# pmgbergen/porepy

Hardware: NVIDIA H100
Metric: 3D cells/sec MPFA+MPSA assembly (higher is better)
Workload: dtype f64

## Files before the change

### porepy_b200/csrc/api.cu

```cuda
#include <cuda_runtime.h>

#include <omp.h>

#include <atomic>
#include <chrono>
#include <thread>
#include <climits>
#include <cstdio>
#include <cstdlib>
#include <cstring>
#include <string>
#include <vector>

#include "csr_build.cuh"
#include <nvtx3/nvToolsExt.h>

struct NvtxRange {
    explicit NvtxRange(const char *name) { nvtxRangePushA(name); }
    ~NvtxRange() { nvtxRangePop(); }
};

static thread_local std::string g_err;
static thread_local int64_t g_err_node = -1;
static std::atomic<int64_t> g_launches{0};

static int fail(int code, const std::string &msg) {
    g_err = msg;
    return code;
}
int pb_fail_(int code, const std::string &msg) { return fail(code, msg); }
void pb_count_launch_() { g_launches++; }

DevPool &pb_dev_pool_() {
    static DevPool *pool = new DevPool;
    return *pool;
}
extern "C" void pb_device_pool_trim(void) { pb_dev_pool_().trim(); }

extern "C" const char *pb_last_error(void) { return g_err.c_str(); }
static std::atomic<int64_t> g_alloc_calls[2];
static std::atomic<int64_t> g_alloc_ns[2];
void pb_alloc_stat_(int kind, double seconds) {
    g_alloc_calls[kind & 1]++;
    g_alloc_ns[kind & 1] += (int64_t)(seconds * 1e9);
}
extern "C" void pb_alloc_stats(double *out) {
    if (!out) return;
    out[0] = (double)g_alloc_calls[0].load(); out[1] = 1e-9 * (double)g_alloc_ns[0].load();
    out[2] = (double)g_alloc_calls[1].load(); out[3] = 1e-9 * (double)g_alloc_ns[1].load();
}
extern "C" int64_t pb_last_error_node(void) { return g_err_node; }
void pb_set_error_node_(int64_t node) { g_err_node = node; }
extern "C" int64_t pb_launch_count(void) { return g_launches.load(); }
extern "C" int pb_device_count(void) {
    int n = 0;
    if (cudaGetDeviceCount(&n) != cudaSuccess) return -1;
    return n;
}
extern "C" int pb_set_device(int device) {
    CUDA_TRY(cudaSetDevice(device));
    return PB_OK;
}

extern "C" int pb_host_alloc(uint64_t bytes, void **out) {
    if (!out) return fail(PB_EINVAL, "null pointer");
    CUDA_TRY(cudaHostAlloc(out, bytes ? bytes : 8, cudaHostAllocDefault));
    return PB_OK;
}
extern "C" void pb_host_free(void *p) {
    if (p) cudaFreeHost(p);
}

static int64_t cfg_scratch(int cfg, int n) {
    switch (cfg) {
        case 0: return Cfg0::scratch_doubles_c();
        case 1: return Cfg1::scratch_doubles_c();
        case 2: return Cfg2::scratch_doubles_c();
        case 3: return Cfg3::scratch_doubles_c();
        case 4: return Cfg4::scratch_doubles_c();
        case 5: return Cfg5::scratch_doubles_c();
        default: return n;
    }
}

static int64_t cfg_pool(int cfg, int n, int w) {
    switch (cfg) {
        case 0: return Cfg0::pool_doubles(n, w);
        case 1: return Cfg1::pool_doubles(n, w);
        case 2: return Cfg2::pool_doubles(n, w);
        case 3: return Cfg3::pool_doubles(n, w);
        case 4: return Cfg4::pool_doubles(n, w);
        case 5: return Cfg5::pool_doubles(n, w);
        default: return Cfg6::pool_doubles(n, w);
    }
}

template <class F>
static int build_classes(pb_plan *p, std::vector<NodeClass> &out, bool rows_to_solver, F size_of) {
    const HostPlan &H = p->H;
    std::vector<int32_t> lists[2 * kNumCfg];
    int64_t amax[2 * kNumCfg] = {0}, rmax[2 * kNumCfg] = {0}, smax[2 * kNumCfg] = {0};
    for (int64_t s = 0; s < H.nn; ++s) {
        int nsc = H.node_sc_ptr[s + 1] - H.node_sc_ptr[s];
        int nsf = H.node_sf_ptr[s + 1] - H.node_sf_ptr[s];
        if (nsf == 0) continue;
        if (!p->active.empty() && !p->active[s]) continue;
        int n = 0, w = 0;
        int64_t a = 0, r = 0;
        size_of(nsf, nsc, H.node_nb[s], &n, &w, &a, &r);
        int cfg = 0;
        while (cfg < kCatchAll && (n > kCfg[cfg].max_n || w > kCfg[cfg].max_w)) ++cfg;
        const int64_t scr = cfg_scratch(cfg, n);
        const int tpb = kCfg[cfg].team == 32 ? 4 : 1;
        bool glob = (size_t)(a + r + scr) * 8 * tpb > kMaxSmem;
        if (glob && (size_t)(r + scr) * 8 * tpb > kMaxSmem)
            return fail(PB_ENOTIMPL, "interaction region at node " + std::to_string(s) +
                                         " is too large for this build (" + std::to_string(nsf) +
                                         " sub-faces)");
        int key = cfg * 2 + (glob ? 1 : 0);
        lists[key].push_back((int32_t)s);
        amax[key] = std::max(amax[key], rows_to_solver ? cfg_pool(cfg, n, w) : a);
        rmax[key] = std::max(rmax[key], r);
        smax[key] = std::max(smax[key], scr);
    }
    out.clear();
    for (int key = 0; key < 2 * kNumCfg; ++key) {
        if (lists[key].empty()) continue;
        out.emplace_back();
        NodeClass &c = out.back();
        c.cfg = key / 2;
        c.a_global = key & 1;
        c.team = kCfg[c.cfg].team;
        c.n = (int)lists[key].size();
        c.a_doubles = amax[key];
        c.rest_doubles = rmax[key];
        c.scr_doubles = smax[key];
        if (!c.a_global) {
            const int tpb = c.team == 32 ? 4 : 1;
            if ((size_t)(c.a_doubles + c.rest_doubles + c.scr_doubles) * 8 * tpb > kMaxSmem) c.a_global = true;
        }
        if (!p->node_key.empty()) {
            const std::vector<uint32_t> &nk = p->node_key;
            std::stable_sort(lists[key].begin(), lists[key].end(), [&](int32_t x, int32_t y) { return nk[x] < nk[y]; });
        }
        if (c.nodes.upload(lists[key], p->stream) != cudaSuccess) return fail(PB_ECUDA, "upload of node list failed");
    }
    return PB_OK;
}

static int build_mpfa_classes(pb_plan *p) {
    const int nd = p->H.nd;
    return build_classes(p, p->mpfa_cls, false, [&](int nsf, int nsc, int nb, int *n, int *w, int64_t *a, int64_t *r) {
        *n = nsf;
        *w = mpfa_width(nd, nsf, nsc, nb);
        *a = mpfa_A_doubles(nd, nsf, nsc, nb);
        *r = mpfa_rest_doubles(nd, nsf, nsc, nb);
    });
}

__global__ void posmap_kernel(int64_t nn, const int32_t *__restrict__ row_ptr, const int32_t *__restrict__ row_ent,
                              const int32_t *__restrict__ col_ptr, const int32_t *__restrict__ col_ent,
                              const int32_t *__restrict__ ip, const int32_t *__restrict__ ix,
                              const int64_t *__restrict__ pos_ptr, int32_t *__restrict__ pos) {
    const int lane = threadIdx.x & 31;
    const int64_t warp = ((int64_t)blockIdx.x * blockDim.x + threadIdx.x) >> 5;
    const int64_t nwarps = ((int64_t)gridDim.x * blockDim.x) >> 5;
    for (int64_t s = warp; s < nn; s += nwarps) {
        const int r0 = row_ptr[s], nr = row_ptr[s + 1] - r0;
        const int c0 = col_ptr[s], ncl = col_ptr[s + 1] - c0;
        const int64_t base = pos_ptr[s];
        for (int e = lane; e < nr * ncl; e += 32) {
            const int i = e / ncl, j = e - i * ncl;
            const int r = row_ent[r0 + i], c = col_ent[c0 + j];
            int lo = ip[r], hi = ip[r + 1];
            while (lo < hi) {
                const int mid = (lo + hi) >> 1;
                if (ix[mid] < c) lo = mid + 1; else hi = mid;
            }
            pos[base + e] = lo;
        }
    }
}

extern "C" int pb_plan_create(int nd, int64_t nc, int64_t nf, int64_t nn, const int32_t *cf_indptr,
                              const int32_t *cf_indices, const int8_t *cf_data,
                              const int32_t *fn_indptr, const int32_t *fn_indices, pb_plan **out) {
    NvtxRange nvtx_("pb_plan_create");
    if (!out || !cf_indptr || !cf_indices || !cf_data || !fn_indptr || !fn_indices)
        return fail(PB_EINVAL, "null pointer");
    int ndev = 0;
    if (cudaGetDeviceCount(&ndev) != cudaSuccess || ndev < 1)
        return fail(PB_ECUDA, "no CUDA device: libporeb200 has no CPU path");
    pb_plan *p = new pb_plan;
    {
        int hw = (int)std::thread::hardware_concurrency();
        const char *lws = getenv("LOCAL_WORLD_SIZE");
        int share = hw / std::max(1, lws ? atoi(lws) : 1);
        const char *ov = getenv("POREB200_PLAN_THREADS");
        int nt = ov ? atoi(ov) : std::min(64, std::max(1, share));
        pb::g_plan_threads = std::max(1, nt);
    }
    auto tp0 = std::chrono::steady_clock::now();
    auto bail = [&](const char *what, cudaError_t e) {
        std::string m = std::string(what) + ": " + cudaGetErrorString(e);
        delete p;
        return fail(PB_ECUDA, m);
    };
    cudaError_t e;
    if ((e = cudaStreamCreateWithFlags(&p->stream, cudaStreamNonBlocking)) != cudaSuccess) return bail("stream", e);
    if ((e = cudaEventCreate(&p->e0)) != cudaSuccess) return bail("event", e);
    if ((e = cudaEventCreate(&p->e1)) != cudaSuccess) return bail("event", e);
    HostPlan &H = p->H;
    cudaStream_t st = p->stream;
    DevBuf fn_idx_dev;
    int rc = getenv("POREB200_HOST_PLAN") ? -1
             : pb_build_device_topology_(p, nd, nc, nf, nn, cf_indptr, cf_indices, cf_data, fn_indptr, fn_indices,
                                         fn_idx_dev);
    if (rc > 0) { delete p; return rc; }
    const bool device_topology = rc == 0;
    if (getenv("POREB200_PLAN_TIMING")) {
        cudaStreamSynchronize(st);
        fprintf(stderr, "[plan] topology on the %s        %8.1f ms (since start)\n", device_topology ? "device" : "host  ",
                std::chrono::duration<double, std::milli>(std::chrono::steady_clock::now() - tp0).count());
    }
    if (!device_topology) {
        p->H = HostPlan{};
        std::string err;
        rc = build_host_plan(nd, nc, nf, nn, cf_indptr, cf_indices, cf_data, fn_indptr, fn_indices,
                             p->H, err, false, false);
        if (rc) {
            delete p;
            return fail(rc, err);
        }
#define UP(field, vec)                                                      \
    if ((e = p->field.upload(vec, st)) != cudaSuccess) return bail(#field, e);
        UP(fn_indptr, H.fn_indptr) UP(node_sc_ptr, H.node_sc_ptr) UP(sc_cell, H.sc_cell)
        UP(node_sf_ptr, H.node_sf_ptr) UP(sf_face, H.sf_face) UP(sf_sides, H.sf_sides)
        UP(sf_bloc, H.sf_bloc) UP(slot_sf, H.slot_sf) UP(node_nb, H.node_nb) UP(sc_ncn, H.sc_ncn)
        UP(posfc_ptr, H.posfc_ptr) UP(posfb_ptr, H.posfb_ptr) UP(poscc_ptr, H.poscc_ptr)
        UP(poscb_ptr, H.poscb_ptr) UP(nbf_ptr, H.nbf_ptr) UP(nbf_idx, H.nbf_idx) UP(cn_ptr, H.cn_ptr)
        UP(cn_idx, H.cn_idx) UP(face_cells, H.face_cells)
#undef UP
        if ((e = fn_idx_dev.upload(fn_indices, (size_t)fn_indptr[nf], st)) != cudaSuccess) return bail("fn_indices", e);
        if ((e = p->cf_ip.upload(cf_indptr, (size_t)nc + 1, st)) != cudaSuccess) return bail("cf_indptr", e);
        if ((e = p->cf_ix.upload(cf_indices, (size_t)cf_indptr[nc], st)) != cudaSuccess) return bail("cf_indices", e);
        if ((e = p->cf_sg.upload(cf_data, (size_t)cf_indptr[nc], st)) != cudaSuccess) return bail("cf_data", e);
    }
    {
        struct PJob { int which; int64_t nrows, ncols; DevBuf *rnp, *rn, *cp, *ci; };
        PJob pj[4] = {{0, nf, nc, &p->fn_indptr, &fn_idx_dev, &p->node_sc_ptr, &p->sc_cell},
                      {1, nf, nf, &p->fn_indptr, &fn_idx_dev, &p->nbf_ptr, &p->nbf_idx},
                      {2, nc, nc, &p->cn_ptr, &p->cn_idx, &p->node_sc_ptr, &p->sc_cell},
                      {3, nc, nf, &p->cn_ptr, &p->cn_idx, &p->nbf_ptr, &p->nbf_idx}};
        DevBuf counts, flag;
        if ((e = flag.ensure(sizeof(int))) != cudaSuccess) return bail("flag", e);
        if ((e = cudaMemsetAsync(flag.p, 0, sizeof(int), st)) != cudaSuccess) return bail("memset", e);
        bool host_fallback = false;
        for (auto &j : pj) {
            DevBuf &ip = p->pat_ip[j.which];
            if ((e = counts.ensure((size_t)j.nrows * sizeof(int32_t))) != cudaSuccess) return bail("counts", e);
            if ((e = ip.ensure((size_t)(j.nrows + 1) * sizeof(int32_t))) != cudaSuccess) return bail("indptr", e);
            const int block = 256;
            int grid = (int)std::max<int64_t>(1, std::min<int64_t>((j.nrows + 7) / 8, (int64_t)pb_sm_count() * 8));
            pattern_kernel<256><<<grid, block, 0, st>>>(j.nrows, j.rnp->as<int32_t>(), j.rn->as<int32_t>(),
                                                        j.cp->as<int32_t>(), j.ci->as<int32_t>(),
                                                        counts.as<int32_t>(), nullptr, nullptr, 0, flag.as<int>());
            g_launches++;
            int ov = 0;
            if ((e = cudaMemcpyAsync(&ov, flag.p, sizeof(ov), cudaMemcpyDeviceToHost, st)) != cudaSuccess) return bail("copy", e);
            int64_t tot = 0;
            if ((rc = pb_scan_offsets_(counts.as<int32_t>(), ip.as<int32_t>(), j.nrows, st, &tot))) { delete p; return rc; }
            if (ov) { host_fallback = true; break; }
            if (tot > 0x7FFFFFFFll) { delete p; return fail(PB_EINVAL, "pattern exceeds 2^31 entries; split the grid"); }
            if ((e = p->pat_idx[j.which].ensure((size_t)std::max<int64_t>(1, tot) * sizeof(int32_t))) != cudaSuccess) return bail("indices", e);
            pattern_kernel<256><<<grid, block, 0, st>>>(j.nrows, j.rnp->as<int32_t>(), j.rn->as<int32_t>(),
                                                        j.cp->as<int32_t>(), j.ci->as<int32_t>(), nullptr,
                                                        ip.as<int32_t>(), p->pat_idx[j.which].as<int32_t>(), 1,
                                                        flag.as<int>());
            g_launches++;
            p->pat_rows[j.which] = j.nrows; p->pat_cols[j.which] = j.ncols; p->pat_nnz[j.which] = tot;
        }
        if (host_fallback) {
            std::string err2;
            HostPlan H2;
            int rc2 = build_host_plan(nd, nc, nf, nn, cf_indptr, cf_indices, cf_data, fn_indptr, fn_indices,
                                      H2, err2, false, true);
            if (rc2) { delete p; return fail(rc2, err2); }
            for (int w = 0; w < 4; ++w) {
                if ((e = p->pat_ip[w].upload(H2.pat[w].indptr, st)) != cudaSuccess) return bail("indptr", e);
                if ((e = p->pat_idx[w].upload(H2.pat[w].indices, st)) != cudaSuccess) return bail("indices", e);
                p->pat_rows[w] = H2.pat[w].nrows; p->pat_cols[w] = H2.pat[w].ncols; p->pat_nnz[w] = H2.pat[w].nnz();
            }
            if ((e = cudaStreamSynchronize(st)) != cudaSuccess) return bail("sync", e);
        }
        if (getenv("POREB200_PLAN_TIMING")) {
            cudaStreamSynchronize(st);
            fprintf(stderr, "[plan] patterns on device done     %8.1f ms (since start)\n",
                    std::chrono::duration<double, std::milli>(std::chrono::steady_clock::now() - tp0).count());
        }
    }
    {
        struct Job { DevBuf *pos; const std::vector<int64_t> *ptr; DevBuf *pptr; int pat;
                     DevBuf *rp, *re, *cp, *ce; };
        Job jobs[4] = {
            {&p->pos_fc, &H.posfc_ptr, &p->posfc_ptr, 0, &p->node_sf_ptr, &p->sf_face, &p->node_sc_ptr, &p->sc_cell},
            {&p->pos_fb, &H.posfb_ptr, &p->posfb_ptr, 1, &p->node_sf_ptr, &p->sf_face, &p->nbf_ptr, &p->nbf_idx},
            {&p->pos_cc, &H.poscc_ptr, &p->poscc_ptr, 2, &p->node_sc_ptr, &p->sc_cell, &p->node_sc_ptr, &p->sc_cell},
            {&p->pos_cb, &H.poscb_ptr, &p->poscb_ptr, 3, &p->node_sc_ptr, &p->sc_cell, &p->nbf_ptr, &p->nbf_idx},
        };
        for (auto &j : jobs) {
            if ((e = j.pos->ensure((size_t)std::max<int64_t>(1, j.ptr->back()) * sizeof(int32_t))) != cudaSuccess)
                return bail("pos map", e);
            const int block = 256;
            int64_t need = (nn * 32 + block - 1) / block;
            int grid = (int)std::max<int64_t>(1, std::min<int64_t>(need, (int64_t)pb_sm_count() * 16));
            posmap_kernel<<<grid, block, 0, st>>>(nn, j.rp->as<int32_t>(), j.re->as<int32_t>(),
                                                  j.cp->as<int32_t>(), j.ce->as<int32_t>(),
                                                  p->pat_ip[j.pat].as<int32_t>(), p->pat_idx[j.pat].as<int32_t>(),
                                                  j.pptr->as<int64_t>(), j.pos->as<int32_t>());
            g_launches++;
            if ((e = cudaGetLastError()) != cudaSuccess) return bail("posmap_kernel", e);
        }
    }
    if ((e = p->err.ensure(sizeof(int))) != cudaSuccess) return bail("err", e);
    PlanView &v = p->view;
    v.nd = nd; v.nc = nc; v.nf = nf; v.nn = nn;
    v.fn_indptr = p->fn_indptr.as<int32_t>();
    v.node_sc_ptr = p->node_sc_ptr.as<int32_t>(); v.sc_cell = p->sc_cell.as<int32_t>();
    v.node_sf_ptr = p->node_sf_ptr.as<int32_t>(); v.sf_face = p->sf_face.as<int32_t>();
    v.sf_sides = p->sf_sides.as<uint32_t>(); v.sf_bloc = p->sf_bloc.as<uint16_t>();
    v.slot_sf = p->slot_sf.as<uint16_t>(); v.node_nb = p->node_nb.as<int32_t>();
    v.sc_ncn = p->sc_ncn.as<int32_t>();
    v.posfc_ptr = p->posfc_ptr.as<int64_t>(); v.posfb_ptr = p->posfb_ptr.as<int64_t>();
    v.poscc_ptr = p->poscc_ptr.as<int64_t>(); v.poscb_ptr = p->poscb_ptr.as<int64_t>();
    v.pos_fc = p->pos_fc.as<int32_t>(); v.pos_fb = p->pos_fb.as<int32_t>();
    v.pos_cc = p->pos_cc.as<int32_t>(); v.pos_cb = p->pos_cb.as<int32_t>();
    v.fc_indptr = p->pat_ip[0].as<int32_t>(); v.fb_indptr = p->pat_ip[1].as<int32_t>();
    v.cc_indptr = p->pat_ip[2].as<int32_t>(); v.cb_indptr = p->pat_ip[3].as<int32_t>();
    rc = build_mpfa_classes(p);
    if (rc) { delete p; return rc; }
    if ((e = cudaStreamSynchronize(st)) != cudaSuccess) return bail("sync", e);
    {
        auto drop = [](auto &v) { v.clear(); v.shrink_to_fit(); };
        drop(H.sc_cell); drop(H.sf_face); drop(H.sf_sides); drop(H.sf_bloc); drop(H.slot_sf); drop(H.sc_ncn);
        drop(H.posfc_ptr); drop(H.posfb_ptr); drop(H.poscc_ptr); drop(H.poscb_ptr);
        drop(H.nbf_ptr); drop(H.nbf_idx); drop(H.cn_ptr); drop(H.cn_idx); drop(H.face_cells); drop(H.fn_indptr);
    }
    if (getenv("POREB200_PLAN_TIMING"))
        fprintf(stderr, "[plan] total incl. upload          %8.1f ms\n",
                std::chrono::duration<double, std::milli>(std::chrono::steady_clock::now() - tp0).count());
    *out = p;
    return PB_OK;
}

extern "C" void pb_plan_destroy(pb_plan *p) {
    if (!p) return;
    if (p->stream) cudaStreamSynchronize(p->stream);
    if (p->e0) cudaEventDestroy(p->e0);
    if (p->e1) cudaEventDestroy(p->e1);
    if (p->stream) cudaStreamDestroy(p->stream);
    delete p;
}

extern "C" int pb_plan_sizes(const pb_plan *p, int64_t *num_subcells, int64_t *num_subfaces,
                             int64_t *num_subhalffaces, int32_t *max_sf, int32_t *max_sc) {
    if (!p) return fail(PB_EINVAL, "null plan");
    if (num_subcells) *num_subcells = p->H.S;
    if (num_subfaces) *num_subfaces = p->H.U;
    if (num_subhalffaces) *num_subhalffaces = p->H.H;
    if (max_sf) *max_sf = p->H.max_nsf;
    if (max_sc) *max_sc = p->H.max_nsc;
    return PB_OK;
}

extern "C" int pb_plan_class_counts(const pb_plan *p, int kind, int64_t *counts) {
    if (!p || !counts) return fail(PB_EINVAL, "null pointer");
    if (kind != 0 && kind != 1) return fail(PB_EINVAL, "kind must be 0 (MPFA) or 1 (MPSA)");
    for (int k = 0; k < 2 * kNumCfg; ++k) counts[k] = 0;
    for (const NodeClass &c : kind == 0 ? p->mpfa_cls : p->mpsa_cls) counts[2 * c.cfg + (c.a_global ? 1 : 0)] += c.n;
    return PB_OK;
}

extern "C" int pb_plan_set_active_nodes(pb_plan *p, const uint8_t *mask) {
    if (!p) return pb_fail_(PB_EINVAL, "null plan");
    if (mask) p->active.assign(mask, mask + p->H.nn); else p->active.clear();
    p->mpsa_cls_nalpha = -1;
    int rc = build_mpfa_classes(p);
    if (rc) return rc;
    CUDA_TRY(cudaStreamSynchronize(p->stream));
    return PB_OK;
}

extern "C" int pb_plan_pattern_size(const pb_plan *p, int which, int64_t *nrows, int64_t *nnz) {
    if (!p || which < 0 || which > 3) return fail(PB_EINVAL, "bad pattern id");
    *nrows = p->pat_rows[which];
    *nnz = p->pat_nnz[which];
    return PB_OK;
}

extern "C" int pb_plan_pattern_get(const pb_plan *p, int which, int32_t *indptr, int32_t *indices) {
    if (!p || which < 0 || which > 3) return fail(PB_EINVAL, "bad pattern id");
    CUDA_TRY(cudaMemcpyAsync(indptr, p->pat_ip[which].p, (p->pat_rows[which] + 1) * sizeof(int32_t), cudaMemcpyDeviceToHost, p->stream));
    if (p->pat_nnz[which])
        CUDA_TRY(cudaMemcpyAsync(indices, p->pat_idx[which].p, p->pat_nnz[which] * sizeof(int32_t),
                                 cudaMemcpyDeviceToHost, p->stream));
    CUDA_TRY(cudaStreamSynchronize(p->stream));
    return PB_OK;
}

__global__ void expand_pattern_kernel(int64_t nrows, const int32_t *__restrict__ ip,
                                      const int32_t *__restrict__ ix, int br, int bc,
                                      int32_t *__restrict__ nip, int32_t *__restrict__ nix) {
    const int lane = threadIdx.x & 31;
    const int64_t warp = ((int64_t)blockIdx.x * blockDim.x + threadIdx.x) >> 5;
    const int64_t nwarps = ((int64_t)gridDim.x * blockDim.x) >> 5;
    for (int64_t r = warp; r < nrows; r += nwarps) {
        const int64_t b = ip[r], len = ip[r + 1] - b;
        const int64_t base = (int64_t)br * bc * b, rowlen = len * bc;
        for (int i = 0; i < br; ++i) {
            if (lane == 0) nip[r * br + i] = (int32_t)(base + i * rowlen);
            for (int64_t t = lane; t < rowlen; t += 32) {
                const int64_t q = t / bc;
                const int j = (int)(t - q * bc);
                nix[base + i * rowlen + t] = ix[b + q] * bc + j;
            }
        }
    }
    if (warp == 0 && lane == 0) nip[nrows * br] = (int32_t)((int64_t)br * bc * ip[nrows]);
}

static int expand_pattern(pb_plan *p, int which, int br, int bc, int32_t *nip, int32_t *nix) {
    const int64_t nrows = p->pat_rows[which];
    const int block = 256;
    int grid = (int)std::max<int64_t>(1, std::min<int64_t>((nrows * 32 + block - 1) / block, (int64_t)pb_sm_count() * 16));
    expand_pattern_kernel<<<grid, block, 0, p->stream>>>(nrows, p->pat_ip[which].as<int32_t>(),
                                                         p->pat_idx[which].as<int32_t>(), br, bc, nip, nix);
    g_launches++;
    CUDA_TRY(cudaGetLastError());
    return PB_OK;
}

extern "C" int pb_plan_pattern_expanded(pb_plan *p, int which, int br, int bc, int32_t *indptr,
                                        int32_t *indices) {
    if (!p || which < 0 || which > 3 || br < 1 || bc < 1 || !indptr || !indices)
        return fail(PB_EINVAL, "bad arguments");
    struct { int64_t nrows, ncols; } c{p->pat_rows[which], p->pat_cols[which]};
    const int64_t nnz = p->pat_nnz[which] * br * bc;
    if (nnz >= 0x7FFFFFFFll || c.ncols * bc >= 0x7FFFFFFFll)
        return fail(PB_ENOTIMPL, "expanded pattern does not fit int32 indices");
    DevBuf nip, nix;
    cudaStream_t st = p->stream;
    CUDA_TRY(nip.ensure((c.nrows * br + 1) * sizeof(int32_t)));
    CUDA_TRY(nix.ensure((nnz ? nnz : 1) * sizeof(int32_t)));
    int rc = expand_pattern(p, which, br, bc, nip.as<int32_t>(), nix.as<int32_t>());
    if (rc) return rc;
// ... 714 lines not shown
```

### porepy_b200/csrc/mpfa_launch.cu

```cuda
#include "assembly_kernels.cuh"

int pb_launch_mpfa_(pb_plan *p, const MpfaParams &prm, const MpfaOut &o) {
    const int nd = p->H.nd;
    for (const NodeClass &c : p->mpfa_cls) {
        int rc = PB_OK;
        if (nd == 3) { PB_LAUNCH_CFG(mpfa_kernel, 3, prm, o) } else { PB_LAUNCH_CFG(mpfa_kernel, 2, prm, o) }
        if (rc) return rc;
    }
    return PB_OK;
}
```

### porepy_b200/csrc/node_kernels.cuh

```cuda
#pragma once
#include <cmath>
#include <cstdint>

#include "views.hpp"

namespace pb {

struct CpuTeam {
    PB_HD int tid() const { return 0; }
    PB_HD int size() const { return 1; }
    PB_HD int lanes() const { return 1; }
    PB_HD int warp() const { return 0; }
    PB_HD int nwarps() const { return 1; }
    PB_HD int lane() const { return 0; }
    PB_HD void sync() const {}
    PB_HD void warp_argmax(double &, int &) const {}
};

#if defined(__CUDACC__)
template <int TEAM>
struct GpuTeam {
    __device__ __forceinline__ int tid() const { return TEAM == 32 ? (threadIdx.x & 31) : threadIdx.x; }
    __device__ __forceinline__ int size() const { return TEAM; }
    __device__ __forceinline__ int lanes() const { return 32; }
// ... 251 lines not shown
                        else {
                            const double f = v[i][j] * rpiv;
#pragma unroll
                            for (int jj = j + 1; jj < 4; ++jj) v[i][jj] -= f * prow[jj];
                        }
                    }
                }
            }
        }
        int prj = -1;
#pragma unroll
        for (int j = 0; j < 4; ++j)
            if (j == mj) prj = mypr[j];
        const double m = (prj >= 0) ? ((mi < pw) ? P0[prj * 4 + mi] : 0.0) : (mi == mj ? 1.0 : 0.0);
        const double growth = invert_block(l, m, iv);
        if (!(growth < 1e300)) sing = true;
        if (l < 16) Ainv[l] = iv;
        if (l == 0) {
#pragma unroll
            for (int j = 0; j < 4; ++j) {
                prs[j] = mypr[j];
                if (mypr[j] >= 0) { usedf[mypr[j]] = 1; rowidx[p0 + j] = mypr[j]; }
            }
            if (sing) prs[4] = 1;
        }
    }


    static PB_HD int x_stride(int nrhs) { return ((nrhs + 11) / 16) * 16 + 4; }
    static constexpr bool kFillTiles = NW > 2;
    static PB_HD int64_t pool_doubles(int n, int W) {
        if (!kFillTiles) return (int64_t)n * W;
        const int64_t x = (int64_t)n * x_stride(W - n), f = (int64_t)NW * 8 * W;
        return x > f ? x : f;
    }

    template <class Team>
    static __device__ __forceinline__ bool solve(Team &t, double *A, int n, int W, int nrhs,
                                                 int *rowidx, double *scratch) {
        const int ti = t.warp(), l = t.lane();
        const int gr = l >> 2, gc = (l & 3) * 2;
        const int wend = n + nrhs;
        double c[RT][NCT][2];
#pragma unroll
        for (int rt = 0; rt < RT; ++rt) {
            const int myrow = 8 * (ti + NW * rt) + gr;
#pragma unroll
            for (int tc = 0; tc < NCT; ++tc) {
                const int col = 8 * tc + gc;
                c[rt][tc][0] = (myrow < n && col < wend) ? A[myrow * W + col] : 0.0;
                c[rt][tc][1] = (myrow < n && col + 1 < wend) ? A[myrow * W + col + 1] : 0.0;
            }
        }
        if (!eliminate(t, c, n, rowidx, scratch)) return false;
        store(t, c, n, nrhs, A + n, W);
        return true;
    }

    template <class Team, class Fill>
    static __device__ __forceinline__ bool solve_rows(Team &t, const Fill &fill, int n, int nrhs, double *pool,
                                                      int *rowidx, double *scratch, const double *&X, int &ldx) {
        const int ti = t.warp(), l = t.lane();
        const int gr = l >> 2, gc = (l & 3) * 2;
        const int wend = n + nrhs;
        const int W = wend | 1;
        if constexpr (!kFillTiles) {
            fill_system(t, fill, n, nrhs, pool, W);
            X = pool + n;
            ldx = W;
            return solve(t, pool, n, W, nrhs, rowidx, scratch);
        }
        double *buf = pool + (int64_t)ti * 8 * W;
        double c[RT][NCT][2];
#pragma unroll
        for (int rt = 0; rt < RT; ++rt)
#pragma unroll
            for (int tc = 0; tc < NCT; ++tc) c[rt][tc][0] = c[rt][tc][1] = 0.0;
#pragma unroll 1
        for (int ps = 0; ps < RT; ++ps) {
            const int r0 = 8 * (ti + NW * ps);
            if (r0 >= n) break;
            for (int i = l; i < 8 * W; i += 32) buf[i] = 0.0;
            __syncwarp();
            if (l < 8 && r0 + l < n) fill(r0 + l, buf + l * W);
            __syncwarp();
            const double *row = buf + gr * W;
            double sum = 0.0;
            for (int cc = l & 3; cc < n; cc += 4) sum += fabs(row[cc]);
            sum += __shfl_xor_sync(0xffffffffu, sum, 1);
            sum += __shfl_xor_sync(0xffffffffu, sum, 2);
            const double is = sum > 0.0 ? 1.0 / sum : 1.0;
            const int myrow = r0 + gr;
#pragma unroll
            for (int rt = 0; rt < RT; ++rt) {
                if (rt == ps && myrow < n) {
#pragma unroll
                    for (int tc = 0; tc < NCT; ++tc) {
                        const int col = 8 * tc + gc;
                        if (col < wend) c[rt][tc][0] = row[col] * is;
                        if (col + 1 < wend) c[rt][tc][1] = row[col + 1] * is;
                    }
                }
            }
            __syncwarp();
        }
        if (!eliminate(t, c, n, rowidx, scratch)) return false;
        ldx = x_stride(nrhs);
        store(t, c, n, nrhs, pool, ldx);
        X = pool;
        return true;
    }

    template <class Team>
    static __device__ __forceinline__ void store(Team &t, const double (&c)[RT][NCT][2], int n, int nrhs,
                                                 double *X, int ldx) {
        const int ti = t.warp(), l = t.lane();
        const int gr = l >> 2, gc = (l & 3) * 2;
#pragma unroll
        for (int rt = 0; rt < RT; ++rt) {
            const int myrow = 8 * (ti + NW * rt) + gr;
#pragma unroll
            for (int tc = 0; tc < NCT; ++tc) {
                const int col = 8 * tc + gc - n;
                if (myrow < n) {
                    if (col >= 0 && col < nrhs) X[myrow * ldx + col] = c[rt][tc][0];
                    if (col + 1 >= 0 && col + 1 < nrhs) X[myrow * ldx + col + 1] = c[rt][tc][1];
                }
            }
        }
        t.sync();
    }

    template <class Team>
    static __device__ __forceinline__ bool eliminate(Team &t, double (&c)[RT][NCT][2], int n, int *rowidx,
                                                     double *scratch) {
        const int ti = t.warp(), l = t.lane();
        const int gr = l >> 2, gc = (l & 3) * 2;
        double *P0 = scratch;
        double *Raw = P0 + NP * 4;
        double *R = Raw + 4 * WP;
        double *Ainv = R + 4 * WP;
        int *prs = (int *)(Ainv + 16 * (NW + 1));
        int *usedf = prs + 8;
        for (int i = t.tid(); i < NP; i += t.size()) usedf[i] = i < n ? 0 : 1;
        for (int i = t.tid(); i < NP * 4; i += t.size()) P0[i] = 0.0;
        if (t.tid() == 0) prs[4] = 0;
        t.sync();
        const int npanel = (n + 3) >> 2;
        bool ok = true;
#pragma unroll
        for (int tcp = 0; tcp < NRT && tcp < NCT; ++tcp) {
            for (int half = 0; half < 2; ++half) {
                const int q = 2 * tcp + half;
                if (q >= npanel || !ok) break;
                const int p0 = 4 * q;
                const int pw = (n - p0) < 4 ? (n - p0) : 4;
                if (((l & 3) >> 1) == half) {
                    const int j0 = 2 * (l & 1);
#pragma unroll
                    for (int rt = 0; rt < RT; ++rt) {
                        const int myrow = 8 * (ti + NW * rt) + gr;
                        P0[myrow * 4 + j0] = c[rt][tcp][0];
                        P0[myrow * 4 + j0 + 1] = c[rt][tcp][1];
                    }
                }
                int myp[RT];
#pragma unroll
                for (int rt = 0; rt < RT; ++rt) {
                    const int myrow = 8 * (ti + NW * rt) + gr;
                    const int j = myrow - p0;
                    myp[rt] = (j >= 0 && j < pw) ? j : -1;
                    if (myp[rt] >= 0) {
#pragma unroll
                        for (int tc = tcp; tc < NCT; ++tc) {
                            Raw[myp[rt] * WP + 8 * tc + gc] = c[rt][tc][0];
                            Raw[myp[rt] * WP + 8 * tc + gc + 1] = c[rt][tc][1];
                        }
                    }
                }
                t.sync();
                double iv;
                const bool fast = try_diagonal_block(l, P0, usedf, p0, pw, iv);
                const double *ainv = Ainv;
                if (fast) {
                    double *mine = Ainv + 16 * (ti + 1);
                    if (l < 16) mine[l] = iv;
                    __syncwarp();
                    ainv = mine;
                } else {
                    t.sync();
                    if (ti == 0) factor_panel<false>(l, P0, usedf, prs, Ainv, rowidx, p0, pw);
                    t.sync();
                    ok = prs[4] == 0;
                    if (!ok) break;
#pragma unroll
                    for (int rt = 0; rt < RT; ++rt) {
                        const int myrow = 8 * (ti + NW * rt) + gr;
                        myp[rt] = -1;
#pragma unroll
                        for (int j = 0; j < 4; ++j)
                            if (prs[j] == myrow) myp[rt] = j;
                        if (myp[rt] >= 0) {
#pragma unroll
                            for (int tc = tcp; tc < NCT; ++tc) {
                                Raw[myp[rt] * WP + 8 * tc + gc] = c[rt][tc][0];
                                Raw[myp[rt] * WP + 8 * tc + gc + 1] = c[rt][tc][1];
                            }
                        }
                    }
                    t.sync();
                }
                for (int col = 8 * tcp + t.tid(); col < NCT * 8; col += t.size()) {
                    double raw[4];
#pragma unroll
                    for (int i = 0; i < 4; ++i) raw[i] = (i < pw) ? Raw[i * WP + col] : 0.0;
#pragma unroll
                    for (int j = 0; j < 4; ++j) {
                        double x = 0.0;
#pragma unroll
                        for (int i = 0; i < 4; ++i) x += ainv[j * 4 + i] * raw[i];
                        R[j * WP + col] = (j < pw) ? x : 0.0;
                    }
                }
                t.sync();
                if (fast && t.tid() < pw) {
                    usedf[p0 + t.tid()] = 1;
                    rowidx[p0 + t.tid()] = p0 + t.tid();
                }
                {
                    const int k = l & 3;
                    const int src = (l & ~3) | (2 * half + (k >> 1));
                    double af[RT];
#pragma unroll
                    for (int rt = 0; rt < RT; ++rt) {
                        const double v0 = __shfl_sync(0xffffffffu, c[rt][tcp][0], src);
                        const double v1 = __shfl_sync(0xffffffffu, c[rt][tcp][1], src);
                        af[rt] = (k < pw) ? -((k & 1) ? v1 : v0) : 0.0;
                    }
                    const double *rb = R + k * WP + (l >> 2);
#pragma unroll
                    for (int tc = tcp; tc < NCT; ++tc) {
                        const double bf = rb[8 * tc];
#pragma unroll
                        for (int rt = 0; rt + 1 < RT; rt += 2) pb_dmma2(c[rt][tc], c[rt + 1][tc], af[rt], af[rt + 1], bf);
                        if (RT & 1) pb_dmma(c[RT - 1][tc], af[RT - 1], bf);
                    }
#pragma unroll
                    for (int rt = 0; rt < RT; ++rt)
                        if (myp[rt] >= 0) {
#pragma unroll
                            for (int tc = tcp; tc < NCT; ++tc) {
                                c[rt][tc][0] = R[myp[rt] * WP + 8 * tc + gc];
                                c[rt][tc][1] = R[myp[rt] * WP + 8 * tc + gc + 1];
                            }
                        }
                }
            }
        }
        t.sync();
        return ok;
    }
};
#endif

#if defined(__CUDACC__)
__device__ __forceinline__ void pb_prefetch_l2(const void *p) {
    asm volatile("prefetch.global.L2 [%0];" ::"l"(p));
}
#endif

template <int ND>
PB_HD bool invert_small(const double (&D)[ND][ND], double (&E)[ND][ND]);

template <>
PB_HD bool invert_small<2>(const double (&D)[2][2], double (&E)[2][2]) {
    double det = D[0][0] * D[1][1] - D[0][1] * D[1][0];
    if (det == 0.0 || !(det == det)) return false;
    double id = 1.0 / det;
    E[0][0] = D[1][1] * id; E[0][1] = -D[0][1] * id;
    E[1][0] = -D[1][0] * id; E[1][1] = D[0][0] * id;
    return true;
}

template <>
PB_HD bool invert_small<3>(const double (&D)[3][3], double (&E)[3][3]) {
    double c00 = D[1][1] * D[2][2] - D[1][2] * D[2][1];
    double c01 = D[1][2] * D[2][0] - D[1][0] * D[2][2];
    double c02 = D[1][0] * D[2][1] - D[1][1] * D[2][0];
    double det = D[0][0] * c00 + D[0][1] * c01 + D[0][2] * c02;
    if (det == 0.0 || !(det == det)) return false;
    double id = 1.0 / det;
    E[0][0] = c00 * id;
    E[1][0] = c01 * id;
    E[2][0] = c02 * id;
    E[0][1] = (D[0][2] * D[2][1] - D[0][1] * D[2][2]) * id;
    E[1][1] = (D[0][0] * D[2][2] - D[0][2] * D[2][0]) * id;
    E[2][1] = (D[0][1] * D[2][0] - D[0][0] * D[2][1]) * id;
    E[0][2] = (D[0][1] * D[1][2] - D[0][2] * D[1][1]) * id;
    E[1][2] = (D[0][2] * D[1][0] - D[0][0] * D[1][2]) * id;
    E[2][2] = (D[0][0] * D[1][1] - D[0][1] * D[1][0]) * id;
    return true;
}

PB_HD int mpfa_width(int nd, int nsf, int nsc, int nb) { return (nsf + nsc + nb + nd * nsc) | 1; }
PB_HD int64_t mpfa_A_doubles(int nd, int nsf, int nsc, int nb) {
    return (int64_t)nsf * mpfa_width(nd, nsf, nsc, nb);
}
PB_HD int64_t mpfa_rest_doubles(int nd, int nsf, int nsc, int nb) {
    (void)nb;
    int64_t d = 2 * (int64_t)nsc * nd * nd + 2 * (int64_t)nsf;
    int64_t ints = nsc + 5 * (int64_t)nsf + (int64_t)nsc * nd;
    return d + (ints + 1) / 2 + 2;
}

template <int ND, class Solver, class Team>
PB_HD void mpfa_node(Team &t, const PlanView &P, const GeoView &G, const MpfaParams &prm,
                     const MpfaOut &o, int64_t s, double *A, double *smd, double *scratch, int *err) {
    const int sc0 = P.node_sc_ptr[s], nsc = P.node_sc_ptr[s + 1] - sc0;
    const int sf0 = P.node_sf_ptr[s], nsf = P.node_sf_ptr[s + 1] - sf0;
    const int nb = P.node_nb[s];
    if (nsf == 0) return;
    const int nrhs = nsc + nb + ND * nsc;
    const int W = (nsf + nrhs) | 1;
    const int64_t nf = P.nf, nc = P.nc, nn = P.nn;
    double *Tk = smd;
    double *Rk = Tk + nsc * ND * ND;
    double *invmf = Rk + nsc * ND * ND;
    double *robw = invmf + nsf;
    int *cell = (int *)(robw + nsf);
    int *face = cell + nsc;
    int *sides = face + nsf;
    int *bloc = sides + nsf;
    int *bcu = bloc + nsf;
    int *rowidx = bcu + nsf;
    int *slot = rowidx + nsf;

    for (int k = t.tid(); k < nsc; k += t.size()) cell[k] = P.sc_cell[sc0 + k];
    for (int i = t.tid(); i < nsc * ND; i += t.size()) slot[i] = P.slot_sf[(int64_t)sc0 * ND + i];
    for (int u = t.tid(); u < nsf; u += t.size()) {
        const int f = P.sf_face[sf0 + u];
        face[u] = f;
        sides[u] = (int)P.sf_sides[sf0 + u];
        const int bl = P.sf_bloc[sf0 + u];
        bloc[u] = (bl == 0xFFFF) ? -1 : bl;
        const double im = 1.0 / (double)(P.fn_indptr[f + 1] - P.fn_indptr[f]);
        invmf[u] = im;
        int code = 0;
        if (bl != 0xFFFF) {
            code = prm.bc[f];
            if (code == 0) code = 2;
        }
        bcu[u] = code;
        robw[u] = (code == 3 && prm.robw) ? prm.robw[f] * G.farea[f] * im : 0.0;
        rowidx[u] = u;
    }
    for (int i = t.tid(); i < nsf * W; i += t.size()) A[i] = 0.0;
    t.sync();

    for (int k = t.tid(); k < nsc; k += t.size()) {
        const int64_t c = cell[k];
        double xc[ND], xs[ND], K[ND][ND], D[ND][ND], R[ND][ND], E[ND][ND];
#pragma unroll
        for (int i = 0; i < ND; ++i) {
            xc[i] = G.ccent[i * G.cell_cs + c * G.cell_es];
            xs[i] = G.nodes[i * G.node_cs + s * G.node_es];
#pragma unroll
            for (int j = 0; j < ND; ++j) K[i][j] = prm.perm[(i * 3 + j) * prm.perm_cs + c * prm.perm_es];
        }
#pragma unroll
        for (int m = 0; m < ND; ++m) {
            const int u = slot[k * ND + m] >> 1;
            const int64_t f = face[u];
            const double e = (bloc[u] >= 0) ? 0.0 : prm.eta;
            double nrm[ND];
#pragma unroll
            for (int i = 0; i < ND; ++i) {
                const double xf = G.fcent[i * G.face_cs + f * G.face_es];
                D[m][i] = xf + e * (xs[i] - xf) - xc[i];
                nrm[i] = G.fnorm[i * G.face_cs + f * G.face_es] * invmf[u];
            }
#pragma unroll
            for (int j = 0; j < ND; ++j) {
                double a = 0.0;
#pragma unroll
                for (int i = 0; i < ND; ++i) a += nrm[i] * K[i][j];
                R[m][j] = a;
            }
        }
        if (!invert_small<ND>(D, E)) flag_singular(err, s);
#pragma unroll
        for (int m = 0; m < ND; ++m)
#pragma unroll
            for (int m2 = 0; m2 < ND; ++m2) {
                double a = 0.0;
#pragma unroll
                for (int q = 0; q < ND; ++q) a += R[m][q] * E[q][m2];
                Tk[k * ND * ND + m * ND + m2] = a;
                Rk[k * ND * ND + m * ND + m2] = R[m][m2];
            }
    }
    t.sync();

    for (int u = t.tid(); u < nsf; u += t.size()) {
        double *row = A + (int64_t)u * W;
        const int code = bcu[u];
        if (code == 1) {
            row[u] = 1.0;
            row[nsf + nsc + bloc[u]] = 1.0;
            continue;
        }
        for (int sd = 0; sd < 2; ++sd) {
            const int side = sd == 0 ? (sides[u] & 0xFFFF) : ((sides[u] >> 16) & 0xFFFF);
            if (side == 0xFFFF) continue;
            const int k = side / ND, m = side - k * ND;
            const double sg = (slot[side] & 1) ? -1.0 : 1.0;
            double tau = 0.0;
#pragma unroll
            for (int m2 = 0; m2 < ND; ++m2) {
                const int u2 = slot[k * ND + m2] >> 1;
                const double tt = sg * Tk[k * ND * ND + m * ND + m2];
                row[u2] += tt;
                tau += tt;
            }
            row[nsf + k] += tau;
#pragma unroll
            for (int j = 0; j < ND; ++j) row[nsf + nsc + nb + k * ND + j] += sg * Rk[k * ND * ND + m * ND + j];
        }
        if (code == 2 || code == 3) row[nsf + nsc + bloc[u]] = -invmf[u];
        if (code == 3) row[u] -= robw[u];
        double sum = 0.0;
        for (int c = 0; c < nsf; ++c) sum += fabs(row[c]);
        if (!(sum > 0.0)) { flag_singular(err, s); continue; }
        const double is = 1.0 / sum;
        for (int c = 0; c < nsf + nrhs; ++c) row[c] *= is;
    }
    t.sync();

    if (!Solver::solve(t, A, nsf, W, nrhs, rowidx, scratch)) {
        if (t.tid() == 0) flag_singular(err, s);
        t.sync();
        return;
    }

    const int32_t *pfc = P.pos_fc + P.posfc_ptr[s];
    const int32_t *pfb = P.pos_fb + P.posfb_ptr[s];
    for (int u = t.warp(); u < nsf; u += t.nwarps()) {
        int side1 = sides[u] & 0xFFFF;
        {
            const int side2 = (sides[u] >> 16) & 0xFFFF;
            if (side2 != 0xFFFF) {
                double n1 = 0.0, n2 = 0.0;
#pragma unroll
                for (int m2 = 0; m2 < ND; ++m2) {
                    n1 += fabs(Tk[side1 * ND + m2]);
                    n2 += fabs(Tk[side2 * ND + m2]);
                }
                if (n2 < n1) side1 = side2;
            }
        }
        const int k1 = side1 / ND, m1 = side1 - k1 * ND;
        const double *T1 = Tk + k1 * ND * ND + m1 * ND;
        const double *R1 = Rk + k1 * ND * ND + m1 * ND;
        const double *xrow[ND];
        double tau1 = 0.0;
#pragma unroll
        for (int m2 = 0; m2 < ND; ++m2) {
            xrow[m2] = A + (int64_t)rowidx[slot[k1 * ND + m2] >> 1] * W + nsf;
            tau1 += T1[m2];
        }
        const double *xu = A + (int64_t)rowidx[u] * W + nsf;
        const double im = invmf[u];
        for (int c = t.lane(); c < nrhs; c += t.lanes()) {
            double fl = 0.0;
#pragma unroll
            for (int m2 = 0; m2 < ND; ++m2) fl -= T1[m2] * xrow[m2][c];
            const double tr = xu[c] * im;
            if (c < nsc) {
                if (c == k1) fl += tau1;
                const int64_t p = pfc[u * nsc + c];
                if (o.flux) red_add(o.flux + p, fl);
                if (o.bpc) red_add(o.bpc + p, tr);
            } else if (c < nsc + nb) {
                const int64_t p = pfb[u * nb + (c - nsc)];
                if (o.bflux) red_add(o.bflux + p, fl);
                if (o.bpf) red_add(o.bpf + p, tr);
            } else {
                const int cc = c - nsc - nb;
                const int k = cc / ND, j = cc - k * ND;
                if (k == k1) fl += R1[j];
                const int64_t p = (int64_t)pfc[u * nsc + k] * ND + j;
                if (o.vs) red_add(o.vs + p, fl);
                if (o.bpvs) red_add(o.bpvs + p, tr);
            }
        }
    }
    t.sync();
}

}
```

Measured before the change: 7.342 million.

## Stream MPFA row assembly into solver and precompute side selection per face

Replaces explicit zeroing, assembly and row-normalisation of the dense local matrix with a row-producer lambda passed to a new Solver::solve_rows, which returns the solution pointer and stride. Per-face side selection and tau are precomputed once into new shared arrays, and the scatter loop batches position-index loads ahead of the red_add writes. Node classes for MPFA are now built with the flag set to true, and optional clock64 phase instrumentation is added. The intent is to drop a full-matrix zeroing and normalisation pass and to overlap index loads with the scatter, at the cost of extra shared memory per node and a dependency on a solver method defined outside this code. Removing row normalisation may change numerical behaviour unless solve_rows performs it.

```diff
diff --git a/porepy_b200/csrc/api.cu b/porepy_b200/csrc/api.cu
--- a/porepy_b200/csrc/api.cu
+++ b/porepy_b200/csrc/api.cu
@@ -150,7 +150,7 @@
 
 static int build_mpfa_classes(pb_plan *p) {
     const int nd = p->H.nd;
-    return build_classes(p, p->mpfa_cls, false, [&](int nsf, int nsc, int nb, int *n, int *w, int64_t *a, int64_t *r) {
+    return build_classes(p, p->mpfa_cls, true, [&](int nsf, int nsc, int nb, int *n, int *w, int64_t *a, int64_t *r) {
         *n = nsf;
         *w = mpfa_width(nd, nsf, nsc, nb);
         *a = mpfa_A_doubles(nd, nsf, nsc, nb);
diff --git a/porepy_b200/csrc/mpfa_launch.cu b/porepy_b200/csrc/mpfa_launch.cu
--- a/porepy_b200/csrc/mpfa_launch.cu
+++ b/porepy_b200/csrc/mpfa_launch.cu
@@ -9,3 +9,15 @@
     }
     return PB_OK;
 }
+
+#if defined(PB_MPFA_PHASES)
+extern "C" int pb_mpfa_phase_cycles(unsigned long long *out, int reset) {
+    CUDA_TRY(cudaDeviceSynchronize());
+    CUDA_TRY(cudaMemcpyFromSymbol(out, pb::pb_mpfa_phase_cyc, sizeof(pb::pb_mpfa_phase_cyc)));
+    if (reset) {
+        static const unsigned long long zero[16][8] = {};
+        CUDA_TRY(cudaMemcpyToSymbol(pb::pb_mpfa_phase_cyc, zero, sizeof(zero)));
+    }
+    return PB_OK;
+}
+#endif
diff --git a/porepy_b200/csrc/node_kernels.cuh b/porepy_b200/csrc/node_kernels.cuh
--- a/porepy_b200/csrc/node_kernels.cuh
+++ b/porepy_b200/csrc/node_kernels.cuh
@@ -577,14 +577,33 @@
     return true;
 }
 
+#if defined(PB_MPFA_PHASES) && defined(__CUDACC__)
+static __device__ unsigned long long pb_mpfa_phase_cyc[16][8];
+#endif
+#if defined(PB_MPFA_PHASES) && defined(__CUDA_ARCH__)
+#define PB_MPFA_STAMP(i) \
+    if (t.tid() == 0) ph_clk[i] = clock64();
+#define PB_MPFA_FLUSH(TEAM, last)                                                                \
+    if (t.tid() == 0) {                                                                          \
+        atomicAdd(&pb_mpfa_phase_cyc[(TEAM) / 32][0], 1ull);                                     \
+        for (int i = 1; i <= (last); ++i)                                                        \
+            atomicAdd(&pb_mpfa_phase_cyc[(TEAM) / 32][i], (unsigned long long)(ph_clk[i] - ph_clk[i - 1])); \
+    }
+#define PB_MPFA_CLOCKS long long ph_clk[8]; PB_MPFA_STAMP(0)
+#else
+#define PB_MPFA_STAMP(i)
+#define PB_MPFA_FLUSH(TEAM, last)
+#define PB_MPFA_CLOCKS
+#endif
+
 PB_HD int mpfa_width(int nd, int nsf, int nsc, int nb) { return (nsf + nsc + nb + nd * nsc) | 1; }
 PB_HD int64_t mpfa_A_doubles(int nd, int nsf, int nsc, int nb) {
     return (int64_t)nsf * mpfa_width(nd, nsf, nsc, nb);
 }
 PB_HD int64_t mpfa_rest_doubles(int nd, int nsf, int nsc, int nb) {
     (void)nb;
-    int64_t d = 2 * (int64_t)nsc * nd * nd + 2 * (int64_t)nsf;
-    int64_t ints = nsc + 5 * (int64_t)nsf + (int64_t)nsc * nd;
+    int64_t d = 2 * (int64_t)nsc * nd * nd + 3 * (int64_t)nsf;
+    int64_t ints = nsc + 6 * (int64_t)nsf + (int64_t)nsc * nd;
     return d + (ints + 1) / 2 + 2;
 }
 
@@ -595,20 +614,21 @@
     const int sf0 = P.node_sf_ptr[s], nsf = P.node_sf_ptr[s + 1] - sf0;
     const int nb = P.node_nb[s];
     if (nsf == 0) return;
+    PB_MPFA_CLOCKS
     const int nrhs = nsc + nb + ND * nsc;
-    const int W = (nsf + nrhs) | 1;
-    const int64_t nf = P.nf, nc = P.nc, nn = P.nn;
     double *Tk = smd;
     double *Rk = Tk + nsc * ND * ND;
     double *invmf = Rk + nsc * ND * ND;
     double *robw = invmf + nsf;
-    int *cell = (int *)(robw + nsf);
+    double *tau1 = robw + nsf;
+    int *cell = (int *)(tau1 + nsf);
     int *face = cell + nsc;
     int *sides = face + nsf;
     int *bloc = sides + nsf;
     int *bcu = bloc + nsf;
     int *rowidx = bcu + nsf;
-    int *slot = rowidx + nsf;
+    int *sidesel = rowidx + nsf;
+    int *slot = sidesel + nsf;
 
     for (int k = t.tid(); k < nsc; k += t.size()) cell[k] = P.sc_cell[sc0 + k];
     for (int i = t.tid(); i < nsc * ND; i += t.size()) slot[i] = P.slot_sf[(int64_t)sc0 * ND + i];
@@ -629,8 +649,8 @@
         robw[u] = (code == 3 && prm.robw) ? prm.robw[f] * G.farea[f] * im : 0.0;
         rowidx[u] = u;
     }
-    for (int i = t.tid(); i < nsf * W; i += t.size()) A[i] = 0.0;
     t.sync();
+    PB_MPFA_STAMP(1)
 
     for (int k = t.tid(); k < nsc; k += t.size()) {
         const int64_t c = cell[k];
@@ -675,14 +695,33 @@
             }
     }
     t.sync();
-
     for (int u = t.tid(); u < nsf; u += t.size()) {
-        double *row = A + (int64_t)u * W;
+        int side1 = sides[u] & 0xFFFF;
+        const int side2 = (sides[u] >> 16) & 0xFFFF;
+        if (side2 != 0xFFFF) {
+            double n1 = 0.0, n2 = 0.0;
+#pragma unroll
+            for (int m2 = 0; m2 < ND; ++m2) {
+                n1 += fabs(Tk[side1 * ND + m2]);
+                n2 += fabs(Tk[side2 * ND + m2]);
+            }
+            if (n2 < n1) side1 = side2;
+        }
+        sidesel[u] = side1;
+        double tau = 0.0;
+#pragma unroll
+        for (int m2 = 0; m2 < ND; ++m2) tau += Tk[side1 * ND + m2];
+        tau1[u] = tau;
+    }
+    PB_MPFA_STAMP(2)
+    PB_MPFA_STAMP(3)
+
+    auto row_of = [&](int u, double *row) {
         const int code = bcu[u];
         if (code == 1) {
             row[u] = 1.0;
             row[nsf + nsc + bloc[u]] = 1.0;
-            continue;
+            return;
         }
         for (int sd = 0; sd < 2; ++sd) {
             const int side = sd == 0 ? (sides[u] & 0xFFFF) : ((sides[u] >> 16) & 0xFFFF);
@@ -703,73 +742,69 @@
         }
         if (code == 2 || code == 3) row[nsf + nsc + bloc[u]] = -invmf[u];
         if (code == 3) row[u] -= robw[u];
-        double sum = 0.0;
-        for (int c = 0; c < nsf; ++c) sum += fabs(row[c]);
-        if (!(sum > 0.0)) { flag_singular(err, s); continue; }
-        const double is = 1.0 / sum;
-        for (int c = 0; c < nsf + nrhs; ++c) row[c] *= is;
-    }
-    t.sync();
-
-    if (!Solver::solve(t, A, nsf, W, nrhs, rowidx, scratch)) {
+    };
+    const double *X;
+    int ldx;
+    if (!Solver::solve_rows(t, row_of, nsf, nrhs, A, rowidx, scratch, X, ldx)) {
         if (t.tid() == 0) flag_singular(err, s);
         t.sync();
         return;
     }
+    PB_MPFA_STAMP(4)
 
     const int32_t *pfc = P.pos_fc + P.posfc_ptr[s];
     const int32_t *pfb = P.pos_fb + P.posfb_ptr[s];
+    constexpr int kBatch = Solver::team > 32 ? 4 : 1;
     for (int u = t.warp(); u < nsf; u += t.nwarps()) {
-        int side1 = sides[u] & 0xFFFF;
-        {
-            const int side2 = (sides[u] >> 16) & 0xFFFF;
-            if (side2 != 0xFFFF) {
-                double n1 = 0.0, n2 = 0.0;
-#pragma unroll
-                for (int m2 = 0; m2 < ND; ++m2) {
-                    n1 += fabs(Tk[side1 * ND + m2]);
-                    n2 += fabs(Tk[side2 * ND + m2]);
-                }
-                if (n2 < n1) side1 = side2;
-            }
-        }
-        const int k1 = side1 / ND, m1 = side1 - k1 * ND;
-        const double *T1 = Tk + k1 * ND * ND + m1 * ND;
-        const double *R1 = Rk + k1 * ND * ND + m1 * ND;
+        const int side1 = sidesel[u];
+        const int k1 = side1 / ND;
+        const double *T1 = Tk + side1 * ND;
+        const double *R1 = Rk + side1 * ND;
         const double *xrow[ND];
-        double tau1 = 0.0;
-#pragma unroll
-        for (int m2 = 0; m2 < ND; ++m2) {
-            xrow[m2] = A + (int64_t)rowidx[slot[k1 * ND + m2] >> 1] * W + nsf;
-            tau1 += T1[m2];
-        }
-        const double *xu = A + (int64_t)rowidx[u] * W + nsf;
+#pragma unroll
+        for (int m2 = 0; m2 < ND; ++m2) xrow[m2] = X + (int64_t)rowidx[slot[k1 * ND + m2] >> 1] * ldx;
+        const double *xu = X + (int64_t)rowidx[u] * ldx;
         const double im = invmf[u];
-        for (int c = t.lane(); c < nrhs; c += t.lanes()) {
-            double fl = 0.0;
-#pragma unroll
-            for (int m2 = 0; m2 < ND; ++m2) fl -= T1[m2] * xrow[m2][c];
-            const double tr = xu[c] * im;
-            if (c < nsc) {
-                if (c == k1) fl += tau1;
-                const int64_t p = pfc[u * nsc + c];
-                if (o.flux) red_add(o.flux + p, fl);
-                if (o.bpc) red_add(o.bpc + p, tr);
-            } else if (c < nsc + nb) {
-                const int64_t p = pfb[u * nb + (c - nsc)];
-                if (o.bflux) red_add(o.bflux + p, fl);
-                if (o.bpf) red_add(o.bpf + p, tr);
-            } else {
-                const int cc = c - nsc - nb;
-                const int k = cc / ND, j = cc - k * ND;
-                if (k == k1) fl += R1[j];
-                const int64_t p = (int64_t)pfc[u * nsc + k] * ND + j;
-                if (o.vs) red_add(o.vs + p, fl);
-                if (o.bpvs) red_add(o.bpvs + p, tr);
+        const double tau = tau1[u];
+        for (int cb = t.lane(); cb < nrhs; cb += kBatch * t.lanes()) {
+            int64_t pp[kBatch];
+#pragma unroll
+            for (int b = 0; b < kBatch; ++b) {
+                const int c = cb + b * t.lanes();
+                pp[b] = 0;
+                if (c < nsc) pp[b] = pfc[u * nsc + c];
+                else if (c < nsc + nb) pp[b] = pfb[u * nb + (c - nsc)];
+                else if (c < nrhs) pp[b] = (int64_t)pfc[u * nsc + (c - nsc - nb) / ND] * ND + (c - nsc - nb) % ND;
+            }
+#pragma unroll
+            for (int b = 0; b < kBatch; ++b) {
+                const int c = cb + b * t.lanes();
+                if (c >= nrhs) break;
+                double fl = 0.0;
+#pragma unroll
+                for (int m2 = 0; m2 < ND; ++m2) fl -= T1[m2] * xrow[m2][c];
+                const double tr = xu[c] * im;
+                const int64_t p = pp[b];
+                if (c < nsc) {
+                    if (c == k1) fl += tau;
+                    if (o.flux) red_add(o.flux + p, fl);
+                    if (o.bpc) red_add(o.bpc + p, tr);
+                } else if (c < nsc + nb) {
+                    if (o.bflux) red_add(o.bflux + p, fl);
+                    if (o.bpf) red_add(o.bpf + p, tr);
+                } else {
+                    const int cc = c - nsc - nb;
+                    const int k = cc / ND, j = cc - k * ND;
+                    if (k == k1) fl += R1[j];
+                    if (o.vs) red_add(o.vs + p, fl);
+                    if (o.bpvs) red_add(o.bpvs + p, tr);
+                }
             }
         }
     }
     t.sync();
-}
-
-}
+    PB_MPFA_STAMP(5)
+    PB_MPFA_FLUSH(Solver::team, 5)
+}
+
+}
```

Measured after the change: 7.403 million (median of 6 runs). No clear change (+0.8%).
